# slinderman/pyglm

Hardware: AMD Instinct MI355X
Metric: Gibbs sweeps/sec (full resample_model) (higher is better)
Workload: dtype f64 (likelihood Gram: exact integer arithmetic on 13 i8 residue planes, CRT back to f64)

## Files before the change

### pyglm_amd/csrc/pgl_i8gram.hip

```cpp
#include "pgl_common.h"
#include <cmath>
#include <type_traits>

namespace {

constexpr int NP = 15;
struct ModTable {
    int p[NP] = {256, 255, 253, 251, 247, 241, 239, 233, 229, 227, 223, 217, 211, 199, 197};
    int w[NP][NP] = {};
    int pinv[NP] = {};
    constexpr ModTable() {
        for (int q = 1; q < NP; ++q) {
            int prod = 1;
            for (int k = 0; k < q; ++k) {
                w[k][q] = prod > p[q] / 2 ? prod - p[q] : prod;
                prod = (prod * (p[k] % p[q])) % p[q];
            }
            int x = 1;
            while ((prod * x) % p[q] != 1) ++x;
            pinv[q] = x;
        }
    }
};
constexpr ModTable MT{};
__constant__ int c_mod[NP] = {256, 255, 253, 251, 247, 241, 239, 233, 229, 227, 223, 217, 211, 199, 197};

typedef int v4i __attribute__((ext_vector_type(4)));
typedef int v16i __attribute__((ext_vector_type(16)));
typedef __attribute__((address_space(3))) void* lds_ptr_t;
typedef const __attribute__((address_space(1))) void* glb_ptr_t;

constexpr int ELEM_BITS = 50;

constexpr int CS_COLS = 16, CS_LANES = 64, CS_G = 8, CS_ROWS = 4;
template <int G, bool WEIGHTED>
__global__ __launch_bounds__(CS_COLS * CS_LANES) void i8_colstats_kernel(const double* __restrict__ X, long ldx, const double* __restrict__ Om,
                                                                        long ldo, int T, int D, double* __restrict__ amax,
                                                                        double* __restrict__ ss) {
    constexpr int CH = CS_LANES * CS_ROWS;
    __shared__ double red[2][CS_LANES][CS_COLS + 1];
    __shared__ double oms[WEIGHTED ? CH : 1][WEIGHTED ? G : 1];
    const int tid = threadIdx.x, cl = tid % CS_COLS, tl = tid / CS_COLS, c = blockIdx.x * CS_COLS + cl;
    const bool live = c < D;
    const int tchunk = ((T + (int)gridDim.y - 1) / (int)gridDim.y + CH - 1) / CH * CH;
    const int tbeg = (int)blockIdx.y * tchunk;
    T = T < tbeg + tchunk ? T : tbeg + tchunk;
    amax += (long)blockIdx.y * G * D;
    ss += (long)blockIdx.y * G * D;
    double m[G], q[G];
#pragma unroll
    for (int g = 0; g < G; ++g) { m[g] = 0.0; q[g] = 0.0; }
    for (int t0 = tbeg; t0 < T; t0 += CH) {
        if (WEIGHTED) {
            __syncthreads();
            for (int e = tid; e < CH * G; e += CS_COLS * CS_LANES) {
                const int t = t0 + e / G;
                oms[e / G][e % G] = t < T ? Om[(long)t * ldo + e % G] : 0.0;
            }
            __syncthreads();
        }
        double x[CS_ROWS];
#pragma unroll
        for (int r = 0; r < CS_ROWS; ++r) {
            const int t = t0 + tl + r * CS_LANES;
            x[r] = (live && t < T) ? X[(long)t * ldx + c] : 0.0;
        }
#pragma unroll
        for (int r = 0; r < CS_ROWS; ++r)
#pragma unroll
            for (int g = 0; g < G; ++g) {
                const double v = WEIGHTED ? x[r] * oms[tl + r * CS_LANES][g] : x[r];
                m[g] = fmax(m[g], fabs(v));
                q[g] = fma(v, v, q[g]);
            }
    }
#pragma unroll
    for (int g = 0; g < G; ++g) {
        __syncthreads();
        red[0][tl][cl] = m[g];
        red[1][tl][cl] = q[g];
        __syncthreads();
        if (tl == 0 && live) {
            double mm = 0.0, qq = 0.0;
            for (int k = 0; k < CS_LANES; ++k) {
                mm = fmax(mm, red[0][k][cl]);
                qq += red[1][k][cl];
            }
            amax[(long)g * D + c] = mm;
            ss[(long)g * D + c] = qq;
        }
    }
}

__global__ __launch_bounds__(256) void i8_scales_kernel(const double* __restrict__ amax, const double* __restrict__ ss, long n, double limit,
                                                        double* __restrict__ scale, int nch) {
    const long k = (long)blockIdx.x * 256 + threadIdx.x;
    if (k >= n) return;
    double a = amax[k], sq = ss[k];
    for (int y = 1; y < nch; ++y) { a = fmax(a, amax[y * n + k]); sq += ss[y * n + k]; }
    const double nrm = sqrt(sq) * (1.0 + 1e-12);
    double s = 1.0;
    if (!(a < HUGE_VAL) || !(nrm < HUGE_VAL)) s = __builtin_nan("");
    else if (a > 0.0) {
        const double nn = nrm > a ? nrm : a;
        int ea, en, el;
        (void)frexp(a, &ea);
        const double mn = frexp(nn, &en), ml = frexp(limit, &el);
        const int e_norm = el - en - (mn > ml ? 1 : 0);
        const int e = min(ELEM_BITS - ea, e_norm);
        s = ldexp(1.0, e);
    }
    scale[k] = s;
}

__global__ __launch_bounds__(256) void i8_colmax_kernel(const double* __restrict__ Om, long ldo, int T, int n, unsigned long long* __restrict__ out) {
    const int c = blockIdx.x * 256 + threadIdx.x;
    if (c >= n) return;
    const int per = (T + (int)gridDim.y - 1) / (int)gridDim.y, t0 = (int)blockIdx.y * per, t1 = min(T, t0 + per);
    unsigned long long m = 0ull;
    for (int t = t0; t < t1; ++t) {
        const unsigned long long v = (unsigned long long)__double_as_longlong(Om[(long)t * ldo + c]) & 0x7fffffffffffffffull;
        m = v > m ? v : m;
    }
    atomicMax(&out[c], m);
}

__global__ __launch_bounds__(256) void i8_scales_bound_kernel(const double* __restrict__ ss, long ldss, const double* __restrict__ ommax,
                                                              const double* __restrict__ xmax, int D, int G, double limit, double inflate,
                                                              double* __restrict__ scale) {
    const long k = (long)blockIdx.x * 256 + threadIdx.x;
    if (k >= (long)G * D) return;
    const int g = (int)(k / D), d = (int)(k % D);
    const double sq = ss[(long)g * ldss + d];
    const double nrm = sqrt(sq) * inflate;
    const double bound = ommax[g] * xmax[d];
    const double a = bound < nrm ? bound : nrm;
    double s = 1.0;
    if (!(nrm < HUGE_VAL)) s = __builtin_nan("");
    else if (a > 0.0) {
        int ea, en, el;
        (void)frexp(a, &ea);
        const double mn = frexp(nrm, &en), ml = frexp(limit, &el);
        const int e_norm = el - en - (mn > ml ? 1 : 0);
        const int e = min(ELEM_BITS - ea, e_norm);
        s = ldexp(1.0, e);
    }
    scale[k] = s;
}

struct PlaneArgs {
    const double* X; long ldx;
    int transposed;
    const double* Om; long ldo;
    const double* scale;
    int8_t* P;
    int T, D, Dq; long Kp; int np;
    unsigned t_base;
};

__device__ __forceinline__ unsigned pgl_mix32(unsigned x) {
    x ^= x >> 16; x *= 0x7feb352du; x ^= x >> 15; x *= 0x846ca68bu; x ^= x >> 16;
    return x;
}
__device__ __forceinline__ double pgl_i8_dither(unsigned t, unsigned d) { return (double)pgl_mix32(t + pgl_mix32(d + 0x9e3779b9u)) * (1.0 / 4294967296.0); }
__device__ __forceinline__ double pgl_round_dither(double y, double u) {
    const double fl = floor(y);
    return fl + (((y - fl) + u >= 1.0) ? 1.0 : 0.0);
}

constexpr int PT_D = 16;
constexpr double MAGIC = 6755399441055744.0;
template <int PT_T>
__global__ __launch_bounds__(PT_T) void i8_planes_kernel(PlaneArgs a, int G) {
    __shared__ double tile[PT_D][PT_T + 1];
    __shared__ double oms[PT_T];
    const int t0 = blockIdx.x * PT_T, d0 = blockIdx.y * PT_D;
    const int tid = threadIdx.x;
    if (a.transposed) {
        const int t = t0 + tid;
#pragma unroll
        for (int dl = 0; dl < PT_D; ++dl) tile[dl][tid] = (t < a.T && d0 + dl < a.D) ? a.X[(long)(d0 + dl) * a.ldx + t] : 0.0;
    } else {
        const int dl = tid & (PT_D - 1), d = d0 + dl;
        for (int tl = tid / PT_D; tl < PT_T; tl += PT_T / PT_D) {
            const int t = t0 + tl;
            tile[dl][tl] = (t < a.T && d < a.D) ? a.X[(long)t * a.ldx + d] : 0.0;
        }
    }
    const int w = tid >> 6, l = tid & 63, r = l >> 2, tb = 64 * w + 16 * (l & 3);
    const long kt = t0 / 64 + w;
    const bool live = kt * 64 < a.Kp;
    const int d = d0 + r;
    const long nkt = a.Kp / 64;
    int8_t* const dst0 = a.P + (((long)blockIdx.y * nkt + kt) << 10) + l * 16;
    const long plane = (long)a.Dq * a.Kp;
    const bool wrow = a.Om && t0 + tid < a.T;
    const double* const omrow = a.Om ? a.Om + (long)(t0 + tid) * a.ldo : nullptr;
    double om_next = wrow ? omrow[0] : 0.0;
    for (int gz = 0; gz < G; ++gz) {
        __syncthreads();
        if (a.Om) oms[tid] = om_next;
        if (gz + 1 < G) om_next = wrow ? omrow[gz + 1] : 0.0;
        __syncthreads();
        if (!live) continue;
        const double scale = d < a.D ? a.scale[(long)gz * a.D + d] : 0.0;
        double v[16], vm[16];
#pragma unroll
        for (int k = 0; k < 16; ++k) {
            const double x = tile[r][tb + k];
            v[k] = a.Om ? rint((x * oms[tb + k]) * scale)
                        : pgl_round_dither(x * scale, pgl_i8_dither(a.t_base + (unsigned)(t0 + tb + k), (unsigned)d));
            vm[k] = v[k] + MAGIC;
        }
        int8_t* dst = dst0 + (long)gz * a.np * plane;
#pragma unroll
        for (int q = 0; q < NP; ++q) {
            if (q < a.np) {
                unsigned b[16];
                if (q == 0) {
#pragma unroll
                    for (int k = 0; k < 16; ++k) b[k] = (unsigned)__double2loint(vm[k]);
                } else {
                    const double pd = (double)MT.p[q], ip = 1.0 / pd;
#pragma unroll
                    for (int k = 0; k < 16; ++k) {
                        const double qq = fma(v[k], ip, MAGIC) - MAGIC;
                        double rr;
                        asm("v_fma_f64 %0, %1, %2, %3" : "=v"(rr) : "s"(-pd), "v"(qq), "v"(vm[k]));
                        b[k] = (unsigned)__double2loint(rr);
                    }
                }
                v4i out;
#pragma unroll
                for (int j = 0; j < 4; ++j) {
                    const unsigned lo = __builtin_amdgcn_perm(b[4 * j + 1], b[4 * j], 0x0c0c0400u);
                    const unsigned hi = __builtin_amdgcn_perm(b[4 * j + 3], b[4 * j + 2], 0x0c0c0400u);
                    out[j] = (int)__builtin_amdgcn_perm(hi, lo, 0x05040100u);
                }
                __builtin_nontemporal_store(out, reinterpret_cast<v4i*>(dst + (long)q * plane));
            }
        }
    }
}

template <int PT_T>
__global__ __launch_bounds__(PT_T) void i8_planes_t_kernel(PlaneArgs a, int G) {
    __shared__ double oms[CS_G][PT_T + 2];
    const int t0 = blockIdx.x * PT_T, d0 = blockIdx.y * PT_D;
    const int tid = threadIdx.x;
    const int w = tid >> 6, l = tid & 63, r = l >> 2, tb = 64 * w + 16 * (l & 3);
    const long kt = t0 / 64 + w;
    const bool live = kt * 64 < a.Kp;
    const int d = d0 + r;
    double x[16];
    {
        const int t = t0 + tb;
        const double* src = a.X + (long)d * a.ldx + t;
        if (live && d < a.D && t + 16 <= a.T) {
#pragma unroll
            for (int k = 0; k < 16; k += 2) {
                const double2 v2 = *reinterpret_cast<const double2*>(src + k);
                x[k] = v2.x; x[k + 1] = v2.y;
            }
        } else {
#pragma unroll
            for (int k = 0; k < 16; ++k) x[k] = (live && d < a.D && t + k < a.T) ? src[k] : 0.0;
        }
    }
    if (a.Om) {
        const int t = t0 + tid;
        const double* src = a.Om + (long)t * a.ldo;
        for (int g = 0; g < G; ++g) oms[g][tid] = t < a.T ? src[g] : 0.0;
        __syncthreads();
    }
    if (!live) return;
    const long nkt = a.Kp / 64;
    int8_t* const dst0 = a.P + (((long)blockIdx.y * nkt + kt) << 10) + l * 16;
    const long plane = (long)a.Dq * a.Kp;
    for (int gz = 0; gz < G; ++gz) {
        const double scale = d < a.D ? a.scale[(long)gz * a.D + d] : 0.0;
        double v[16], vm[16];
#pragma unroll
        for (int k = 0; k < 16; ++k) {
            v[k] = a.Om ? rint((x[k] * oms[gz][tb + k]) * scale)
                        : pgl_round_dither(x[k] * scale, pgl_i8_dither(a.t_base + (unsigned)(t0 + tb + k), (unsigned)d));
            vm[k] = v[k] + MAGIC;
        }
        int8_t* dst = dst0 + (long)gz * a.np * plane;
#pragma unroll
        for (int q = 0; q < NP; ++q) {
            if (q < a.np) {
                unsigned b[16];
                if (q == 0) {
#pragma unroll
                    for (int k = 0; k < 16; ++k) b[k] = (unsigned)__double2loint(vm[k]);
                } else {
                    const double pd = (double)MT.p[q], ip = 1.0 / pd;
#pragma unroll
                    for (int k = 0; k < 16; ++k) {
                        const double qq = fma(v[k], ip, MAGIC) - MAGIC;
                        double rr;
                        asm("v_fma_f64 %0, %1, %2, %3" : "=v"(rr) : "s"(-pd), "v"(qq), "v"(vm[k]));
                        b[k] = (unsigned)__double2loint(rr);
                    }
                }
                v4i out;
#pragma unroll
                for (int j = 0; j < 4; ++j) {
                    const unsigned lo = __builtin_amdgcn_perm(b[4 * j + 1], b[4 * j], 0x0c0c0400u);
                    const unsigned hi = __builtin_amdgcn_perm(b[4 * j + 3], b[4 * j + 2], 0x0c0c0400u);
                    out[j] = (int)__builtin_amdgcn_perm(hi, lo, 0x05040100u);
                }
                __builtin_nontemporal_store(out, reinterpret_cast<v4i*>(dst + (long)q * plane));
            }
        }
    }
}

constexpr int BKB = 64;
constexpr int KCH = 2000;
constexpr int CH = 32;
constexpr int SB = 6;

struct GramArgs {
    const int8_t* PA;
    const int8_t* PB;
    int8_t* R;
    int Dq; long Kp; int G; int np;
    int sbr, sbc;
    int nkt;
    int kt0;
    int* sched;
    long KpA; int ka0;
    int accum;
    int8_t* Rx;
#ifdef PGL_AB
#define PGL_KPARTS(g_) ((g_).kparts)
#else
#define PGL_KPARTS(g_) 0
#endif
    int kparts;
};

__device__ __forceinline__ int isqrt_tri_i(int t) {
    int r = (int)((__builtin_sqrt(8.0 * (double)t + 1.0) - 1.0) * 0.5);
    while ((long)(r + 1) * (r + 2) / 2 <= t) ++r;
    while ((long)r * (r + 1) / 2 > t) --r;
    return r;
}

__device__ __forceinline__ void clustered_tile(int t, int ntm, int sbr, int sbc, int& tm, int& tn) {
    const int nbr = (ntm + sbr - 1) / sbr;
    for (int I = 0; I < nbr; ++I) {
        const int r0 = I * sbr, r1 = min(ntm, r0 + sbr);
        const int nbc = (r1 - 1) / sbc + 1;
        for (int jj = 0; jj < nbc; ++jj) {
            const int J = (I & 1) ? nbc - 1 - jj : jj;
            const int c0 = J * sbc, c1 = min(ntm, c0 + sbc);
            for (int r = max(r0, c0); r < r1; ++r) {
                const int cnt = min(c1, r + 1) - c0;
                if (t < cnt) { tm = r; tn = c0 + t; return; }
                t -= cnt;
            }
        }
    }
    tm = tn = 0;
}

__device__ __forceinline__ int chunk_swz(int qd) { return (0x1320 >> (4 * qd)) & 3; }

constexpr int BT = 320, BROWS = 2 * BT;
constexpr int BSTAGE = BROWS * BKB;

template <int IDX>
__device__ __forceinline__ void big_mfma(v4i& acc, const v4i& a, const v4i& b) {
    if constexpr (IDX < 64) asm volatile("v_mfma_i32_16x16x64_i8 %0, %1, %2, %0" : "+a"(acc) : "v"(a), "v"(b));
    else asm volatile("v_mfma_i32_16x16x64_i8 %0, %1, %2, %0" : "+v"(acc) : "v"(a), "v"(b));
}

#ifndef PGL_I8_SNAKE
#define PGL_I8_SNAKE 1
#endif
template <bool TRI, int I, int J, typename F>
__device__ __forceinline__ void big_rows(v4i (&acc)[10][10], v4i (&FA)[5], v4i (&FB)[10], F&& slot) {
    if constexpr (I < 10) {
        constexpr int JJ = (PGL_I8_SNAKE && (I & 1) && I != 9) ? 9 - J : J;
        if constexpr (!TRI || JJ <= I) big_mfma<I * 10 + JJ>(acc[I][JJ], FA[I % 5], FB[JJ]);
        slot(std::integral_constant<int, I>{}, std::integral_constant<int, J>{});
        __builtin_amdgcn_sched_barrier(0);
        if constexpr (J == 9) big_rows<TRI, I + 1, 0>(acc, FA, FB, slot);
        else big_rows<TRI, I, J + 1>(acc, FA, FB, slot);
    }
}

constexpr int BNST = 3;
__device__ __forceinline__ void i8_gram_item_big(const GramArgs& g, const int gz, const int q, const int tm, const int tn, char* lds, const int kpart = -1) {
    const int m0 = tm * BT, n0 = tn * BT;
    const int tid = threadIdx.x, lane = tid & 63, wave = tid >> 6;
    const int wm = wave >> 1, wn = wave & 1;
    const long plane = (long)g.Dq * g.Kp;
    const int8_t* A = g.PA + (long)q * g.Dq * g.KpA + (long)g.ka0 * 1024;
    const int8_t* B = g.PB + ((long)gz * g.np + q) * plane;
    const int nkt = g.nkt;
    const int wv = __builtin_amdgcn_readfirstlane(wave);
    const unsigned voff = (unsigned)((lane >> 2) * 64 + (((lane & 3) ^ chunk_swz((lane >> 4) & 3)) * 16));
    const int fr = lane & 15, fc = lane >> 4;
    auto frag = [&](int stage, int row) {
        const int pc = fc ^ chunk_swz((row >> 2) & 3);
        return *reinterpret_cast<const v4i*>(lds + stage * BSTAGE + row * BKB + pc * 16);
    };
    auto rdA = [&](int stage, int f) { return frag(stage, wm * 160 + f * 16 + fr); };
    auto rdB = [&](int stage, int f) { return frag(stage, BT + wn * 160 + f * 16 + fr); };
    const double pq = (double)c_mod[q], ipq = 1.0 / pq;
    auto reduce = [&](int v) {
        const double x = (double)v;
        return (int)fma(-pq, rint(x * ipq), x);
    };
    const bool inplace = PGL_KPARTS(g) > 0;
    int8_t* R = (kpart > 0 && !inplace) ? g.Rx + ((long)gz * 3 + (kpart - 1)) * g.Dq * g.Dq : g.R + ((long)gz * g.np + q) * g.Dq * g.Dq;
    {
        int kc = g.kt0;
        int nk = min(nkt - kc, KCH);
        if (kpart >= 0) {
            const int parts = inplace ? PGL_KPARTS(g) : 4;
            const int quarter = (nk + parts - 1) / parts, kend = kc + nk;
            kc += kpart * quarter;
            nk = min(quarter, kend - kc);
            if (nk <= 0) {
                if (inplace && kpart > 0) return;
                if (g.kt0 == 0 && !g.accum)
                    for (int e = threadIdx.x; e < BT * BT; e += 256) R[(long)(m0 + e / BT) * g.Dq + n0 + e % BT] = 0;
                return;
            }
        }
        const char* sb[10];
#pragma unroll
        for (int i = 0; i < 10; ++i) {
            const int rq = wv + 4 * i;
            const int8_t* base = rq < 20 ? A + (long)(m0 + 16 * rq) * g.KpA : B + (long)(n0 + 16 * (rq - 20)) * g.Kp;
            sb[i] = reinterpret_cast<const char*>(base) + (long)kc * 1024;
        }
        long gadv = nk >= 2 ? 1024 : 0;
        auto dma_piece = [&](int stage, int i) {
            __builtin_amdgcn_global_load_lds((glb_ptr_t)(sb[i] + voff), (lds_ptr_t)(lds + stage * BSTAGE + (wv + 4 * i) * 1024), 16, 0, 0);
            sb[i] += gadv;
        };
#pragma unroll
        for (int i = 0; i < 10; ++i) dma_piece(0, i);
        if (nk < 3) gadv = 0;
#pragma unroll
        for (int i = 0; i < 10; ++i) dma_piece(1, i);
        asm volatile("s_waitcnt vmcnt(10)" ::: "memory");
        __builtin_amdgcn_s_barrier();
        asm volatile("" ::: "memory");
        if (tm == tn && wv == 1) {
            int cur = 0;
            for (int kt = 0; kt < nk; ++kt) {
                const int dst = cur == 0 ? BNST - 1 : cur - 1;
                if (kt + BNST >= nk) gadv = 0;
                asm volatile("s_waitcnt vmcnt(0)" ::: "memory");
                __builtin_amdgcn_s_barrier();
                asm volatile("" ::: "memory");
#pragma unroll
                for (int i = 0; i < 10; ++i) dma_piece(dst, i);
                cur = cur == BNST - 1 ? 0 : cur + 1;
            }
            asm volatile("s_waitcnt vmcnt(0)" ::: "memory");
            __builtin_amdgcn_s_barrier();
            return;
        }
        v4i acc[10][10];
#pragma unroll
        for (int i = 0; i < 10; ++i)
#pragma unroll
            for (int j = 0; j < 10; ++j) acc[i][j] = v4i{0, 0, 0, 0};
        v4i FA[5], FB[10];
#pragma unroll
        for (int f = 0; f < 10; ++f) FB[f] = rdB(0, f);
        FA[0] = rdA(0, 0);
        FA[1] = rdA(0, 1);
        asm volatile("s_nop 7\n\ts_nop 7" ::: "memory");
        auto k_loop = [&](auto tri_c) {
        constexpr bool TRI = decltype(tri_c)::value;
        int cur = 0;
        for (int kt = 0; kt < nk; ++kt) {
            const int nxt = cur == BNST - 1 ? 0 : cur + 1;
            const int dst = cur == 0 ? BNST - 1 : cur - 1;
            if (kt + BNST >= nk) gadv = 0;
            big_rows<TRI, 0, 0>(acc, FA, FB, [&](auto ic, auto jc) {
                constexpr int I = decltype(ic)::value, J = decltype(jc)::value;
                if constexpr (J == 1) { if constexpr (I + 2 < 10) FA[(I + 2) % 5] = rdA(cur, I + 2); else FA[(I + 2) % 5] = rdA(nxt, I + 2 - 10); }
                if constexpr (I == 4 && J == 0) {
                    asm volatile("s_waitcnt vmcnt(0)" ::: "memory");
                    __builtin_amdgcn_s_barrier();
                    asm volatile("" ::: "memory");
                }
                if constexpr (I >= 4 && I <= 8 && (J == 3 || J == 7)) dma_piece(dst, 2 * (I - 4) + (J == 7));
                if constexpr (I == 9 && J >= 1) FB[J - 1] = rdB(nxt, J - 1);
            });
            FB[9] = rdB(nxt, 9);
            cur = nxt;
        }
        };
        if (tm == tn && wm == wn) k_loop(std::true_type{});
        else k_loop(std::false_type{});
        asm volatile("s_waitcnt vmcnt(0)\n\ts_nop 7\n\ts_nop 7\n\ts_nop 7" ::: "memory");
        __builtin_amdgcn_s_barrier();
        auto store = [&](auto accum_c) {
            constexpr bool ACCUM = decltype(accum_c)::value;
#pragma unroll
            for (int i = 0; i < 10; ++i)
#pragma unroll
                for (int j = 0; j < 10; ++j)
#pragma unroll
                    for (int r = 0; r < 4; ++r) {
                        const int row = m0 + wm * 160 + i * 16 + 4 * (lane >> 4) + r;
                        const int col = n0 + wn * 160 + j * 16 + (lane & 15);
                        int8_t* dst8 = R + (long)row * g.Dq + col;
                        int v = reduce(acc[i][j][r]);
                        if constexpr (ACCUM) v = reduce(v + (int)*dst8);
                        *dst8 = (int8_t)(v & 0xff);
                    }
        };
        if (g.kt0 == 0 && !g.accum && !(inplace && kpart > 0)) store(std::false_type{});
        else store(std::true_type{});
    }
}

__global__ __launch_bounds__(256) void i8_gram_kernel(GramArgs g) {
    extern __shared__ __attribute__((aligned(16))) char lds[];
    int* ticket = reinterpret_cast<int*>(lds);
    const int ntm = g.Dq / BT;
    const int ntiles = ntm * (ntm + 1) / 2;
    const int npx = (g.G % 8 == 0) ? g.G / 8 : 0;
    const bool split = npx > 0 && g.Rx != nullptr && PGL_KPARTS(g) == 0;
    const bool pieces = npx > 0 && PGL_KPARTS(g) > 0;
    const int nfull = pieces ? 0 : ntiles * npx * (split ? g.np - 1 : g.np);
    const int per_xcd = pieces ? g.np * PGL_KPARTS(g) * npx * ntiles : nfull + (split ? 4 * ntiles * npx : 0);
    const int total = ntiles * g.np * g.G;
    unsigned xcc;
    asm volatile("s_getreg_b32 %0, hwreg(HW_REG_XCC_ID)" : "=s"(xcc));
    xcc &= 7u;
    for (;;) {
        __syncthreads();
        if (threadIdx.x == 0) {
            int w = -1, y = 0;
            for (int hop = 0; hop < 8 && w < 0; ++hop) {
                y = (int)((xcc + hop) & 7u);
                const int it = atomicAdd(&g.sched[y], 1);
                if (npx) { if (it < per_xcd) w = it; }
                else {
                    const long cand = ((long)(it / CH) * 8 + y) * CH + it % CH;
                    if (cand < total) w = (int)cand;
                }
            }
            if (w >= 0) {
                int tm, tn, gz, q, kpart = -1, tile;
                if (!npx) { const int pair = w / ntiles; tile = w % ntiles; gz = pair / g.np; q = pair % g.np; }
                else if (pieces) {
                    const int per_piece = npx * ntiles, per_plane = PGL_KPARTS(g) * per_piece, r = w % per_plane, r2 = r % per_piece;
                    q = w / per_plane; kpart = r / per_piece; gz = y + 8 * (r2 / ntiles); tile = r2 % ntiles;
                }
                else if (w < nfull) {
                    const int per_plane = npx * ntiles, r = w % per_plane;
                    q = w / per_plane; gz = y + 8 * (r / ntiles); tile = r % ntiles;
                } else {
                    const int r0 = w - nfull, j = r0 / (4 * ntiles), r = r0 % (4 * ntiles), grp = r / 128, within = r - grp * 128;
                    const int tg = min(32, ntiles - grp * 32);
                    kpart = within / tg;
                    tile = grp * 32 + within % tg;
                    gz = y + 8 * j; q = g.np - 1;
                }
                clustered_tile(tile, ntm, g.sbr, g.sbc, tm, tn);
                ticket[1] = gz; ticket[2] = tm; ticket[3] = tn; ticket[4] = kpart; ticket[5] = q;
            }
            ticket[0] = w;
        }
        __syncthreads();
        if (ticket[0] < 0) break;
        const int gz = __builtin_amdgcn_readfirstlane(ticket[1]), q = __builtin_amdgcn_readfirstlane(ticket[5]);
        const int tm = __builtin_amdgcn_readfirstlane(ticket[2]), tn = __builtin_amdgcn_readfirstlane(ticket[3]);
        const int kpart = __builtin_amdgcn_readfirstlane(ticket[4]);
        __syncthreads();
        i8_gram_item_big(g, gz, q, tm, tn, lds, kpart);
    }
}

struct CrtArgs {
    const int8_t* R;
    const double* sA; const double* sB;
    double* J; long ldj; long strideJ;
    int D, Dq, G, accumulate, np;
    const int8_t* Rx;
};

__device__ __forceinline__ double recip_scale(double x) {
    const long long b = __double_as_longlong(x);
    const bool pow2 = (b & 0x000FFFFFFFFFFFFFll) == 0 && b > 0x0010000000000000ll && b < 0x7FD0000000000000ll;
    return pow2 ? __longlong_as_double(0x7FE0000000000000ll - b) : 1.0 / x;
}

__global__ __launch_bounds__(256) void i8_crt_kernel(CrtArgs a) {
    const int j0 = (blockIdx.x * 256 + threadIdx.x) * 4, i = blockIdx.y, gz = blockIdx.z;
    if (j0 > i || i >= a.D) return;
    const int8_t* R = a.R + ((long)gz * a.np) * a.Dq * a.Dq + (long)i * a.Dq + j0;
    int w[NP];
#pragma unroll
    for (int q = 0; q < NP; ++q) w[q] = q < a.np ? *reinterpret_cast<const int*>(R + (long)q * a.Dq * a.Dq) : 0;
    int wx[3] = {0, 0, 0};
    if (a.Rx) {
        const int8_t* Rx = a.Rx + (long)gz * 3 * a.Dq * a.Dq + (long)i * a.Dq + j0;
#pragma unroll
        for (int k = 0; k < 3; ++k) wx[k] = *reinterpret_cast<const int*>(Rx + (long)k * a.Dq * a.Dq);
    }
    const double ra = recip_scale(a.sA[i]);
    double out[4];
#pragma unroll
    for (int e = 0; e < 4; ++e) {
        int v[NP];
#pragma unroll
        for (int q = 0; q < NP; ++q) v[q] = (int)(int8_t)((unsigned)w[q] >> (8 * e));
        if (a.Rx) {
            const int x = (int)(int8_t)((unsigned)wx[0] >> (8 * e)) + (int)(int8_t)((unsigned)wx[1] >> (8 * e)) + (int)(int8_t)((unsigned)wx[2] >> (8 * e));
#pragma unroll
            for (int q = 1; q < NP; ++q) if (q == a.np - 1) v[q] += x;
        }
#pragma unroll
        for (int q = 1; q < NP; ++q) {
            if (q < a.np) {
                const int p = MT.p[q];
                int u = v[q];
#pragma unroll
                for (int k = 0; k < q; ++k) u -= v[k] * MT.w[k][q];
                int t = u * MT.pinv[q] % p;
                if (t > p / 2) t -= p; else if (t < -(p / 2)) t += p;
                v[q] = t;
            }
        }
        double s = 0.0;
#pragma unroll
        for (int q = NP - 1; q >= 0; --q)
            if (q < a.np) s = s * (double)MT.p[q] + (double)v[q];
        const int j = j0 + e;
        const double rb = j < a.D ? recip_scale(a.sB[(long)gz * a.D + j]) : 0.0;
        out[e] = (s * ra) * rb;
    }
    double* dst = a.J + (long)gz * a.strideJ + (long)i * a.ldj + j0;
    if (j0 + 3 <= i && !a.accumulate && (reinterpret_cast<uintptr_t>(dst) % 16 == 0)) {
        *reinterpret_cast<d2_t*>(dst) = d2_t{out[0], out[1]};
        *reinterpret_cast<d2_t*>(dst + 2) = d2_t{out[2], out[3]};
    } else {
#pragma unroll
        for (int e = 0; e < 4; ++e)
            if (j0 + e <= i) dst[e] = a.accumulate ? dst[e] + out[e] : out[e];
    }
}

}

int pgl_k_i8_padded_rows(int D) { return (D + BT - 1) / BT * BT; }

static long pgl_i8_kp(int T) { const long k = ((long)T + 63) / 64 * 64; return k < 256 ? 256 : k; }

double pgl_k_i8_norm_limit(int nplanes, int T) {
    double l2 = 0.0;
    for (int q = 0; q < nplanes && q < NP; ++q) l2 += std::log2((double)MT.p[q]);
    const double lim = (std::exp2((l2 - 1.0) * 0.5) - std::sqrt((double)(T < 1 ? 1 : T)) - 1.0) / (1.0 + 1e-9);
    return lim > 0.0 ? lim : 0.0;
}
int pgl_k_i8_nu(int nplanes, int T) {
    const double lim = pgl_k_i8_norm_limit(nplanes, T);
    if (!(lim >= 2.0)) return 0;
    return (int)std::floor(std::log2(lim) - 1e-12);
}
int pgl_k_i8_max_planes(void) { return NP; }
int pgl_k_i8_min_planes(int T) {
    for (int k = 1; k <= NP; ++k)
        if (pgl_k_i8_nu(k, T) >= 50) return k;
    return NP + 1;
}

long pgl_k_i8_kp(int T) { return pgl_i8_kp(T); }
static int pgl_k_i8_kparts() { static const int v = pgl_ab_int("PGL_I8_KPARTS", 0); return v >= 2 && v <= 16 ? v : 0; }
static bool pgl_k_i8_split(int G, int nplanes) { return G % 8 == 0 && nplanes >= 2 && pgl_k_i8_kparts() == 0; }
size_t pgl_k_i8_plane_bytes(int D, int T) {
    const long Dq = pgl_k_i8_padded_rows(D), Kp = pgl_i8_kp(T);
    return (size_t)NP * Dq * Kp;
}
size_t pgl_k_i8_residue_bytes(int D) {
    const long Dq = pgl_k_i8_padded_rows(D);
    return (size_t)NP * Dq * Dq;
}

int pgl_k_i8_colstats(const double* X, long ldx, const double* Om, long ldo, int T, int D, int G, double* amax, double* ss, hipStream_t st) {
    if (G > CS_G || G < 1) { pgl_set_error("i8 colstats: %d weight columns per call (max %d)", G, CS_G); return PGL_ERR_ARG; }
    const dim3 grid((D + CS_COLS - 1) / CS_COLS), block(CS_COLS * CS_LANES);
#define PGL_CS(g_) case g_: hipLaunchKernelGGL((i8_colstats_kernel<g_, true>), grid, block, 0, st, X, ldx, Om, ldo, T, D, amax, ss); break;
    if (!Om) hipLaunchKernelGGL((i8_colstats_kernel<1, false>), grid, block, 0, st, X, ldx, Om, ldo, T, D, amax, ss);
    else switch (G) { PGL_CS(1) PGL_CS(2) PGL_CS(3) PGL_CS(4) PGL_CS(5) PGL_CS(6) PGL_CS(7) PGL_CS(8) default: break; }
#undef PGL_CS
    PGL_CHECK_LAUNCH();
    return PGL_OK;
}

constexpr int CS_NCH = 4;
int pgl_k_i8_colstats_scales(const double* X, long ldx, const double* Om, long ldo, int T, int D, int G, int nplanes, double* scratch, double* scale,
                             hipStream_t st) {
    if (G > CS_G || G < 1 || !Om) { pgl_set_error("i8 colstats+scales: %d weight columns per call (max %d)", G, CS_G); return PGL_ERR_ARG; }
    if (pgl_k_i8_nu(nplanes, T) < 8) { pgl_set_error("i8 scales: %d moduli leave no room for T = %d", nplanes, T); return PGL_ERR_ARG; }
    const int nch = T >= 4096 ? CS_NCH : 1;
    double* pm = scratch;
    double* pq = scratch + (size_t)CS_NCH * G * D;
    const dim3 grid((D + CS_COLS - 1) / CS_COLS, nch), block(CS_COLS * CS_LANES);
#define PGL_CS2(g_) case g_: hipLaunchKernelGGL((i8_colstats_kernel<g_, true>), grid, block, 0, st, X, ldx, Om, ldo, T, D, pm, pq); break;
    switch (G) { PGL_CS2(1) PGL_CS2(2) PGL_CS2(3) PGL_CS2(4) PGL_CS2(5) PGL_CS2(6) PGL_CS2(7) PGL_CS2(8) default: break; }
#undef PGL_CS2
    PGL_CHECK_LAUNCH();
    const long n = (long)G * D;
    hipLaunchKernelGGL(i8_scales_kernel, dim3((unsigned)((n + 255) / 256)), dim3(256), 0, st, pm, pq, n, pgl_k_i8_norm_limit(nplanes, T), scale, nch);
    PGL_CHECK_LAUNCH();
    return PGL_OK;
}

int pgl_k_i8_colmax(const double* Om, long ldo, int T, int n, double* out, hipStream_t st) {
    if (hipMemsetAsync(out, 0, (size_t)n * sizeof(double), st) != hipSuccess) { pgl_set_error("memset failed"); return PGL_ERR_HIP; }
    hipLaunchKernelGGL(i8_colmax_kernel, dim3((unsigned)((n + 255) / 256), (unsigned)(T >= 8192 ? 128 : 1)), dim3(256), 0, st, Om, ldo, T, n,
                       reinterpret_cast<unsigned long long*>(out));
    PGL_CHECK_LAUNCH();
    return PGL_OK;
}

int pgl_k_i8_scales_bound(const double* ss, long ldss, const double* ommax, const double* xmax, int D, int G, int T, int nplanes, double* scale,
                          hipStream_t st) {
    if (pgl_k_i8_nu(nplanes, T) < 8) { pgl_set_error("i8 scales: %d moduli leave no room for T = %d", nplanes, T); return PGL_ERR_ARG; }
    const long n = (long)G * D;
    hipLaunchKernelGGL(i8_scales_bound_kernel, dim3((unsigned)((n + 255) / 256)), dim3(256), 0, st, ss, ldss, ommax, xmax, D, G,
                       pgl_k_i8_norm_limit(nplanes, T), 1.0 + ((double)T + 16.0) * 1.2e-16, scale);
    PGL_CHECK_LAUNCH();
    return PGL_OK;
}

int pgl_k_i8_scales(const double* amax, const double* ss, long n, int T, int nplanes, double* scale, hipStream_t st) {
    if (pgl_k_i8_nu(nplanes, T) < 8) { pgl_set_error("i8 scales: %d moduli leave no room for T = %d", nplanes, T); return PGL_ERR_ARG; }
    hipLaunchKernelGGL(i8_scales_kernel, dim3((unsigned)((n + 255) / 256)), dim3(256), 0, st, amax, ss, n, pgl_k_i8_norm_limit(nplanes, T), scale, 1);
    PGL_CHECK_LAUNCH();
    return PGL_OK;
}

int pgl_k_i8_planes(const double* X, long ldx, int transposed, const double* Om, long ldo, const double* scale, int8_t* P, int T, int D, int G,
                    int nplanes, long t_base, hipStream_t st) {
    const int Dq = pgl_k_i8_padded_rows(D);
    const long Kp = pgl_i8_kp(T);
    const bool aligned = (ldx % 2 == 0) && (reinterpret_cast<uintptr_t>(X) % 16 == 0);
    for (int g0 = 0; g0 < G; g0 += CS_G) {
        const int gz = G - g0 < CS_G ? G - g0 : CS_G;
        PlaneArgs a{X, ldx, transposed, Om ? Om + g0 : nullptr, ldo, scale + (long)g0 * D, P + (long)g0 * nplanes * Dq * Kp, T, D, Dq, Kp, nplanes, (unsigned)t_base};
        if (transposed && aligned)
            hipLaunchKernelGGL(i8_planes_t_kernel<256>, dim3((unsigned)((Kp + 255) / 256), Dq / PT_D), dim3(256), 0, st, a, gz);
        else
            hipLaunchKernelGGL(i8_planes_kernel<512>, dim3((unsigned)((Kp + 511) / 512), Dq / PT_D), dim3(512), 0, st, a, gz);
        PGL_CHECK_LAUNCH();
    }
    return PGL_OK;
}

int pgl_k_i8_gram(const int8_t* PA, long KpA, int ka0, const int8_t* PB, int8_t* R, int8_t* Rx, int T, int D, int G, int nplanes, int accumulate, hipStream_t st) {
    const int Dq = pgl_k_i8_padded_rows(D);
    const long Kp = pgl_i8_kp(T);
    if (KpA <= 0) { KpA = Kp; ka0 = 0; }
    const int nkt = (T + BKB - 1) / BKB;
    if (KpA % BKB != 0 || (long)(ka0 + nkt) * BKB > KpA) { pgl_set_error("i8 gram: slice of %d tiles at tile %d outside the X planes (%ld bytes per row)", nkt, ka0, KpA); return PGL_ERR_ARG; }
    static PglPerDevice attr;
    if (int rc = pgl_set_dynamic_lds(reinterpret_cast<const void*>(i8_gram_kernel), BNST * BSTAGE, attr)) return rc;
    const int n_cu = pgl_device_cus(pgl_device());
    const int ntm = Dq / BT, ntiles = ntm * (ntm + 1) / 2;
    const long total = (long)ntiles * nplanes * G;
    if (total <= 0) return PGL_OK;
    if (total * 4 > 0x7fffffffL) { pgl_set_error("i8 gram: %ld work items", total); return PGL_ERR_ARG; }
    const unsigned grid = (unsigned)(total < n_cu ? total : n_cu);
    const bool lists = G % 8 == 0;
    static const int sbr_ab = pgl_ab_int("PGL_I8_SBR", 0), sbc_ab = pgl_ab_int("PGL_I8_SBC", 0);
    const int sbr = sbr_ab > 0 ? sbr_ab : (lists ? ntm : SB), sbc = sbc_ab > 0 ? sbc_ab : (lists ? 2 : SB);
    for (int kt0 = 0; kt0 < nkt; kt0 += KCH) {
        GramArgs g{PA, PB, R, Dq, Kp, G, nplanes, sbr, sbc, nkt, kt0, pgl_sched_slot(st), KpA, ka0, accumulate ? 1 : 0, pgl_k_i8_split(G, nplanes) ? Rx : nullptr, lists ? pgl_k_i8_kparts() : 0};
        if (!g.sched) { pgl_set_error("i8 gram: scheduler scratch unavailable"); return PGL_ERR_HIP; }
        hipLaunchKernelGGL(i8_gram_kernel, dim3(grid), dim3(256), BNST * BSTAGE, st, g);
        PGL_CHECK_LAUNCH();
    }
    return PGL_OK;
}

int pgl_k_i8_crt(const int8_t* R, const int8_t* Rx, const double* sA, const double* sB, double* J, long ldj, long strideJ, int D, int G, int nplanes,
                 int accumulate, hipStream_t st) {
    const int Dq = pgl_k_i8_padded_rows(D);
    if (G <= 0) return PGL_OK;
    CrtArgs c{R, sA, sB, J, ldj, strideJ, D, Dq, G, accumulate, nplanes, (Rx != nullptr && pgl_k_i8_split(G, nplanes)) ? Rx : nullptr};
    hipLaunchKernelGGL(i8_crt_kernel, dim3((D + 1023) / 1024, D, G), dim3(256), 0, st, c);
    PGL_CHECK_LAUNCH();
    return PGL_OK;
}
```

Measured before the change: 0.05820.

## Compute i8 residues with packed 16-bit ops and float CRT over lower-triangle grid

New measurement: 0.05838, median of 6. Within noise of the previous version (+0.3%).

```diff
diff --git a/pyglm_amd/csrc/pgl_i8gram.hip b/pyglm_amd/csrc/pgl_i8gram.hip
--- a/pyglm_amd/csrc/pgl_i8gram.hip
+++ b/pyglm_amd/csrc/pgl_i8gram.hip
@@ -7,18 +7,22 @@
 constexpr int NP = 15;
 struct ModTable {
     int p[NP] = {256, 255, 253, 251, 247, 241, 239, 233, 229, 227, 223, 217, 211, 199, 197};
+    int pinv[NP] = {};
     int w[NP][NP] = {};
-    int pinv[NP] = {};
     constexpr ModTable() {
         for (int q = 1; q < NP; ++q) {
+            const int m = p[q];
             int prod = 1;
+            for (int k = 0; k < q; ++k) prod = (prod * (p[k] % m)) % m;
+            int x = 1;
+            while ((prod * x) % m != 1) ++x;
+            pinv[q] = x > m / 2 ? x - m : x;
+            prod = 1;
             for (int k = 0; k < q; ++k) {
-                w[k][q] = prod > p[q] / 2 ? prod - p[q] : prod;
-                prod = (prod * (p[k] % p[q])) % p[q];
-            }
-            int x = 1;
-            while ((prod * x) % p[q] != 1) ++x;
-            pinv[q] = x;
+                const int t = (prod * x) % m;
+                w[k][q] = t > m / 2 ? t - m : t;
+                prod = (prod * (p[k] % m)) % m;
+            }
         }
     }
 };
@@ -170,7 +174,38 @@
 
 constexpr int PT_D = 16;
 constexpr double MAGIC = 6755399441055744.0;
-template <int PT_T>
+typedef unsigned short v2us __attribute__((ext_vector_type(2)));
+
+template <bool STORE_ONLY>
+__device__ __forceinline__ void i8_store_residues(const double (&v)[16], int8_t* dst, long plane, int np) {
+    unsigned lo[8];
+#pragma unroll
+    for (int j = 0; j < 8; ++j)
+        lo[j] = __builtin_amdgcn_perm((unsigned)__double2loint(v[2 * j + 1] + MAGIC), (unsigned)__double2loint(v[2 * j] + MAGIC), 0x05040100u);
+#pragma unroll
+    for (int q = 0; q < NP; ++q) {
+        if (q < np) {
+            unsigned r[8];
+#pragma unroll
+            for (int j = 0; j < 8; ++j) {
+                r[j] = lo[j];
+                if (q > 0 && !STORE_ONLY) {
+                    const double ip = 1.0 / (double)MT.p[q];
+                    const unsigned qq = __builtin_amdgcn_perm((unsigned)__double2loint(fma(v[2 * j + 1], ip, MAGIC)),
+                                                              (unsigned)__double2loint(fma(v[2 * j], ip, MAGIC)), 0x05040100u);
+                    const v2us m = {(unsigned short)(65536 - MT.p[q]), (unsigned short)(65536 - MT.p[q])};
+                    r[j] = __builtin_bit_cast(unsigned, (v2us)(__builtin_bit_cast(v2us, qq) * m + __builtin_bit_cast(v2us, lo[j])));
+                }
+            }
+            v4i out;
+#pragma unroll
+            for (int j = 0; j < 4; ++j) out[j] = (int)__builtin_amdgcn_perm(r[2 * j + 1], r[2 * j], 0x06040200u);
+            __builtin_nontemporal_store(out, reinterpret_cast<v4i*>(dst + (long)q * plane));
+        }
+    }
+}
+
+template <int PT_T, bool STORE_ONLY>
 __global__ __launch_bounds__(PT_T) void i8_planes_kernel(PlaneArgs a, int G) {
     __shared__ double tile[PT_D][PT_T + 1];
     __shared__ double oms[PT_T];
@@ -204,46 +239,18 @@
         __syncthreads();
         if (!live) continue;
         const double scale = d < a.D ? a.scale[(long)gz * a.D + d] : 0.0;
-        double v[16], vm[16];
+        double v[16];
 #pragma unroll
         for (int k = 0; k < 16; ++k) {
             const double x = tile[r][tb + k];
             v[k] = a.Om ? rint((x * oms[tb + k]) * scale)
                         : pgl_round_dither(x * scale, pgl_i8_dither(a.t_base + (unsigned)(t0 + tb + k), (unsigned)d));
-            vm[k] = v[k] + MAGIC;
-        }
-        int8_t* dst = dst0 + (long)gz * a.np * plane;
-#pragma unroll
-        for (int q = 0; q < NP; ++q) {
-            if (q < a.np) {
-                unsigned b[16];
-                if (q == 0) {
-#pragma unroll
-                    for (int k = 0; k < 16; ++k) b[k] = (unsigned)__double2loint(vm[k]);
-                } else {
-                    const double pd = (double)MT.p[q], ip = 1.0 / pd;
-#pragma unroll
-                    for (int k = 0; k < 16; ++k) {
-                        const double qq = fma(v[k], ip, MAGIC) - MAGIC;
-                        double rr;
-                        asm("v_fma_f64 %0, %1, %2, %3" : "=v"(rr) : "s"(-pd), "v"(qq), "v"(vm[k]));
-                        b[k] = (unsigned)__double2loint(rr);
-                    }
-                }
-                v4i out;
-#pragma unroll
-                for (int j = 0; j < 4; ++j) {
-                    const unsigned lo = __builtin_amdgcn_perm(b[4 * j + 1], b[4 * j], 0x0c0c0400u);
-                    const unsigned hi = __builtin_amdgcn_perm(b[4 * j + 3], b[4 * j + 2], 0x0c0c0400u);
-                    out[j] = (int)__builtin_amdgcn_perm(hi, lo, 0x05040100u);
-                }
-                __builtin_nontemporal_store(out, reinterpret_cast<v4i*>(dst + (long)q * plane));
-            }
-        }
-    }
-}
-
-template <int PT_T>
+        }
+        i8_store_residues<STORE_ONLY>(v, dst0 + (long)gz * a.np * plane, plane, a.np);
+    }
+}
+
+template <int PT_T, bool STORE_ONLY>
 __global__ __launch_bounds__(PT_T) void i8_planes_t_kernel(PlaneArgs a, int G) {
     __shared__ double oms[CS_G][PT_T + 2];
     const int t0 = blockIdx.x * PT_T, d0 = blockIdx.y * PT_D;
@@ -279,41 +286,12 @@
     const long plane = (long)a.Dq * a.Kp;
     for (int gz = 0; gz < G; ++gz) {
         const double scale = d < a.D ? a.scale[(long)gz * a.D + d] : 0.0;
-        double v[16], vm[16];
-#pragma unroll
-        for (int k = 0; k < 16; ++k) {
+        double v[16];
+#pragma unroll
+        for (int k = 0; k < 16; ++k)
             v[k] = a.Om ? rint((x[k] * oms[gz][tb + k]) * scale)
                         : pgl_round_dither(x[k] * scale, pgl_i8_dither(a.t_base + (unsigned)(t0 + tb + k), (unsigned)d));
-            vm[k] = v[k] + MAGIC;
-        }
-        int8_t* dst = dst0 + (long)gz * a.np * plane;
-#pragma unroll
-        for (int q = 0; q < NP; ++q) {
-            if (q < a.np) {
-                unsigned b[16];
-                if (q == 0) {
-#pragma unroll
-                    for (int k = 0; k < 16; ++k) b[k] = (unsigned)__double2loint(vm[k]);
-                } else {
-                    const double pd = (double)MT.p[q], ip = 1.0 / pd;
-#pragma unroll
-                    for (int k = 0; k < 16; ++k) {
-                        const double qq = fma(v[k], ip, MAGIC) - MAGIC;
-                        double rr;
-                        asm("v_fma_f64 %0, %1, %2, %3" : "=v"(rr) : "s"(-pd), "v"(qq), "v"(vm[k]));
-                        b[k] = (unsigned)__double2loint(rr);
-                    }
-                }
-                v4i out;
-#pragma unroll
-                for (int j = 0; j < 4; ++j) {
-                    const unsigned lo = __builtin_amdgcn_perm(b[4 * j + 1], b[4 * j], 0x0c0c0400u);
-                    const unsigned hi = __builtin_amdgcn_perm(b[4 * j + 3], b[4 * j + 2], 0x0c0c0400u);
-                    out[j] = (int)__builtin_amdgcn_perm(hi, lo, 0x05040100u);
-                }
-                __builtin_nontemporal_store(out, reinterpret_cast<v4i*>(dst + (long)q * plane));
-            }
-        }
+        i8_store_residues<STORE_ONLY>(v, dst0 + (long)gz * a.np * plane, plane, a.np);
     }
 }
 
@@ -600,40 +578,41 @@
     return pow2 ? __longlong_as_double(0x7FE0000000000000ll - b) : 1.0 / x;
 }
 
+constexpr int CRT_COLS = 1024;
 __global__ __launch_bounds__(256) void i8_crt_kernel(CrtArgs a) {
-    const int j0 = (blockIdx.x * 256 + threadIdx.x) * 4, i = blockIdx.y, gz = blockIdx.z;
+    int band = 0, rem = (int)blockIdx.x;
+    while (rem >= CRT_COLS * (band + 1)) { rem -= CRT_COLS * (band + 1); ++band; }
+    const int i = band * CRT_COLS + rem / (band + 1), gz = blockIdx.y;
+    const int j0 = ((rem % (band + 1)) * 256 + threadIdx.x) * 4;
     if (j0 > i || i >= a.D) return;
     const int8_t* R = a.R + ((long)gz * a.np) * a.Dq * a.Dq + (long)i * a.Dq + j0;
-    int w[NP];
-#pragma unroll
-    for (int q = 0; q < NP; ++q) w[q] = q < a.np ? *reinterpret_cast<const int*>(R + (long)q * a.Dq * a.Dq) : 0;
-    int wx[3] = {0, 0, 0};
+    unsigned w[NP];
+#pragma unroll
+    for (int q = 0; q < NP; ++q) w[q] = q < a.np ? *reinterpret_cast<const unsigned*>(R + (long)q * a.Dq * a.Dq) ^ 0x80808080u : 0x80808080u;
+    unsigned wx[3] = {0x80808080u, 0x80808080u, 0x80808080u};
     if (a.Rx) {
         const int8_t* Rx = a.Rx + (long)gz * 3 * a.Dq * a.Dq + (long)i * a.Dq + j0;
 #pragma unroll
-        for (int k = 0; k < 3; ++k) wx[k] = *reinterpret_cast<const int*>(Rx + (long)k * a.Dq * a.Dq);
+        for (int k = 0; k < 3; ++k) wx[k] = *reinterpret_cast<const unsigned*>(Rx + (long)k * a.Dq * a.Dq) ^ 0x80808080u;
     }
     const double ra = recip_scale(a.sA[i]);
     double out[4];
 #pragma unroll
     for (int e = 0; e < 4; ++e) {
-        int v[NP];
-#pragma unroll
-        for (int q = 0; q < NP; ++q) v[q] = (int)(int8_t)((unsigned)w[q] >> (8 * e));
-        if (a.Rx) {
-            const int x = (int)(int8_t)((unsigned)wx[0] >> (8 * e)) + (int)(int8_t)((unsigned)wx[1] >> (8 * e)) + (int)(int8_t)((unsigned)wx[2] >> (8 * e));
-#pragma unroll
-            for (int q = 1; q < NP; ++q) if (q == a.np - 1) v[q] += x;
-        }
+        const auto residue = [e](unsigned word) { return (float)((word >> (8 * e)) & 0xffu); };
+        const float x = (residue(wx[0]) + residue(wx[1]) + residue(wx[2])) - 384.0f;
+        float v[NP];
+        v[0] = residue(w[0]) - 128.0f;
 #pragma unroll
         for (int q = 1; q < NP; ++q) {
             if (q < a.np) {
-                const int p = MT.p[q];
-                int u = v[q];
-#pragma unroll
-                for (int k = 0; k < q; ++k) u -= v[k] * MT.w[k][q];
-                int t = u * MT.pinv[q] % p;
-                if (t > p / 2) t -= p; else if (t < -(p / 2)) t += p;
+                const float p = (float)MT.p[q], pinv = (float)MT.pinv[q], half = (float)(MT.p[q] / 2);
+                float u = fmaf(residue(w[q]), pinv, -128.0f * pinv);
+                if (a.Rx && q == a.np - 1) u = fmaf(x, pinv, u);
+#pragma unroll
+                for (int k = 0; k < q; ++k) u = fmaf(v[k], -(float)MT.w[k][q], u);
+                float t = fmaf(-p, __builtin_rintf(u * (1.0f / p)), u);
+                t = t > half ? t - p : t < -half ? t + p : t;
                 v[q] = t;
             }
         }
@@ -755,10 +734,18 @@
     for (int g0 = 0; g0 < G; g0 += CS_G) {
         const int gz = G - g0 < CS_G ? G - g0 : CS_G;
         PlaneArgs a{X, ldx, transposed, Om ? Om + g0 : nullptr, ldo, scale + (long)g0 * D, P + (long)g0 * nplanes * Dq * Kp, T, D, Dq, Kp, nplanes, (unsigned)t_base};
+#ifdef PGL_AB
+        static const bool store_only = pgl_ab_int("PGL_I8_PLANES_STORE_ONLY", 0) != 0;
+        if (store_only && transposed && aligned) {
+            hipLaunchKernelGGL((i8_planes_t_kernel<256, true>), dim3((unsigned)((Kp + 255) / 256), Dq / PT_D), dim3(256), 0, st, a, gz);
+            PGL_CHECK_LAUNCH();
+            continue;
+        }
+#endif
         if (transposed && aligned)
-            hipLaunchKernelGGL(i8_planes_t_kernel<256>, dim3((unsigned)((Kp + 255) / 256), Dq / PT_D), dim3(256), 0, st, a, gz);
+            hipLaunchKernelGGL((i8_planes_t_kernel<256, false>), dim3((unsigned)((Kp + 255) / 256), Dq / PT_D), dim3(256), 0, st, a, gz);
         else
-            hipLaunchKernelGGL(i8_planes_kernel<512>, dim3((unsigned)((Kp + 511) / 512), Dq / PT_D), dim3(512), 0, st, a, gz);
+            hipLaunchKernelGGL((i8_planes_kernel<512, false>), dim3((unsigned)((Kp + 511) / 512), Dq / PT_D), dim3(512), 0, st, a, gz);
         PGL_CHECK_LAUNCH();
     }
     return PGL_OK;
@@ -795,7 +782,10 @@
     const int Dq = pgl_k_i8_padded_rows(D);
     if (G <= 0) return PGL_OK;
     CrtArgs c{R, sA, sB, J, ldj, strideJ, D, Dq, G, accumulate, nplanes, (Rx != nullptr && pgl_k_i8_split(G, nplanes)) ? Rx : nullptr};
-    hipLaunchKernelGGL(i8_crt_kernel, dim3((D + 1023) / 1024, D, G), dim3(256), 0, st, c);
+    long blocks = 0;
+    for (int i0 = 0; i0 < D; i0 += CRT_COLS) blocks += (long)(D - i0 < CRT_COLS ? D - i0 : CRT_COLS) * (i0 / CRT_COLS + 1);
+    if (blocks > 0x7fffffffL || G > 65535) { pgl_set_error("i8 crt: %ld blocks x %d neurons", blocks, G); return PGL_ERR_ARG; }
+    hipLaunchKernelGGL(i8_crt_kernel, dim3((unsigned)blocks, (unsigned)G), dim3(256), 0, st, c);
     PGL_CHECK_LAUNCH();
     return PGL_OK;
 }
```
